# rafaelsoStanford/State_Policy_DiffusionModel

Hardware: AMD Instinct MI355X
Metric: denoise-steps/sec (B=4096, horizon=32) (higher is better)
Workload: dtype f32 (split-fp16 MFMA operands, fp32 accumulate)

## Files before the change

include/spdm.h:

```cpp
#ifndef SPDM_H
#define SPDM_H

#include <stddef.h>
#include <stdint.h>

#ifdef __cplusplus
extern "C" {
#endif

#define SPDM_NAME_MAX 64
#define SPDM_ABI_VERSION 2

typedef enum {
    SPDM_OK = 0,
    SPDM_ERR_INVALID = -1,
    SPDM_ERR_HIP = -2,
    SPDM_ERR_STATE = -3,
    SPDM_ERR_MISSING = -4,
    SPDM_ERR_NOMEM = -5
} spdm_status;

typedef enum { SPDM_DDPM = 0, SPDM_DDIM = 1 } spdm_scheduler_kind;

typedef struct spdm_handle spdm_handle;
// ... 89 lines not shown

typedef struct spdm_encoder spdm_encoder;
int  spdm_encoder_create(int32_t device, const float* h_blob, size_t n_floats, const spdm_tensor_index* h_index,
                         int32_t n_index, spdm_encoder** out);
int  spdm_encoder_forward(spdm_encoder* e, int32_t n_images, const float* d_images, float* d_latent, void* stream);
void spdm_encoder_destroy(spdm_encoder* e);

int  spdm_debug_geometry(int32_t M, int32_t N, int32_t K, int32_t HW, int32_t W, int32_t taps, uint32_t switches,
                         int32_t out[10]);

int  spdm_op_gelu(const float* d_x, float* d_y, size_t n, void* stream);

typedef struct {
    int32_t B, H, W, K, N, taps;
    int32_t split;
    int32_t pro;
    int32_t epi;
    const float* d_src;  int32_t src_ld;
    const float* d_skip; int32_t skip_ld;  int32_t up_C;
    const float* h_weight;
    const double* d_src_stats; int32_t src_slots, src_m_tile, src_n_tiles, src_cnorm;
    const float* d_gamma; const float* d_beta;
    const double* d_skip_stats; int32_t skip_slots, skip_m_tile, skip_n_tiles, skip_cnorm;
    const float* d_skip_gamma; const float* d_skip_beta;
    const float* d_bias; const float* d_resid; int32_t resid_ld;
    float* d_dst; int32_t dst_ld;
    double* d_stats; size_t stats_cap;
    double* d_row_stats; size_t row_stats_cap;
    int32_t out[10];
} spdm_op_gemm_args;

int  spdm_op_gemm(spdm_op_gemm_args* args);

#ifdef __cplusplus
}
#endif
#endif
```

state_policy_diffusionmodel_amd/_lib.py:

```python
from __future__ import annotations

import ctypes
import os
from ctypes import POINTER, c_char_p, c_double, c_float, c_int32, c_int64, c_size_t, c_uint64, c_void_p

from .weights import TensorIndex

HERE = os.path.dirname(os.path.abspath(__file__))
LIB_PATH = os.environ.get("SPDM_LIB") or os.path.join(HERE, "libspdm_hip.so")

SPDM_DDPM, SPDM_DDIM = 0, 1
SPDM_FLAG_DEBUG_KEEP = 1
SPDM_FLAG_EXACT_FP32 = 2
SPDM_FLAG_SIMPLE_UNET = 4
SPDM_FLAG_TRAIN = 8
SPDM_FLAG_TRAIN_ATTENTION = 16
ABI_VERSION = 2


class SpdmOpGemmArgs(ctypes.Structure):
    _fields_ = ([(n, c_int32) for n in ("B", "H", "W", "K", "N", "taps", "split", "pro", "epi")] +
                [("d_src", c_void_p), ("src_ld", c_int32), ("d_skip", c_void_p), ("skip_ld", c_int32), ("up_C", c_int32),
                 ("h_weight", c_void_p),
                 ("d_src_stats", c_void_p)] + [(n, c_int32) for n in ("src_slots", "src_m_tile", "src_n_tiles", "src_cnorm")] +
                [("d_gamma", c_void_p), ("d_beta", c_void_p),
                 ("d_skip_stats", c_void_p)] + [(n, c_int32) for n in ("skip_slots", "skip_m_tile", "skip_n_tiles", "skip_cnorm")] +
                [("d_skip_gamma", c_void_p), ("d_skip_beta", c_void_p),
                 ("d_bias", c_void_p), ("d_resid", c_void_p), ("resid_ld", c_int32),
                 ("d_dst", c_void_p), ("dst_ld", c_int32),
                 ("d_stats", c_void_p), ("stats_cap", c_size_t), ("d_row_stats", c_void_p), ("row_stats_cap", c_size_t),
                 ("out", c_int32 * 10)])


class SpdmConfig(ctypes.Structure):
    _fields_ = [(n, c_int32) for n in ("horizon", "state_dim", "cond_dim", "time_dim", "attention", "max_batch",
                                        "device", "num_train_timesteps", "flags")]


SYMBOLS = {
    "spdm_abi_version": (c_int32, []),
    "spdm_last_error": (c_char_p, []),
    "spdm_create": (c_int32, [POINTER(SpdmConfig), POINTER(c_void_p)]),
    "spdm_destroy": (None, [c_void_p]),
    "spdm_load_weights": (c_int32, [c_void_p, c_void_p, c_size_t, POINTER(TensorIndex), c_int32]),
    "spdm_set_time_table": (c_int32, [c_void_p, c_void_p, c_int32]),
    "spdm_set_schedule": (c_int32, [c_void_p, c_int32, c_int32, c_int32, c_float, c_float]),
    "spdm_set_schedule_tables": (c_int32, [c_void_p, c_int32, c_int32, c_void_p, c_void_p]),
    "spdm_schedule_tables": (c_int32, [c_int32, c_int32, c_int32, c_float, c_float, c_void_p, c_void_p]),
    "spdm_unet_forward": (c_int32, [c_void_p, c_int32, c_void_p, c_void_p, c_int32, c_void_p, c_void_p, c_void_p]),
    "spdm_sample": (c_int32, [c_void_p, c_int32, c_void_p, c_void_p, c_int32, c_int32, c_void_p, c_void_p, c_uint64,
                              c_uint64, c_void_p, c_void_p, c_void_p]),
    "spdm_train_loss_grad": (c_int32, [c_void_p, c_int32, c_void_p, c_void_p, c_int32, c_void_p, c_void_p, c_void_p, c_void_p,
                                       c_void_p, c_void_p, c_void_p]),
    "spdm_sample_begin": (c_int32, [c_void_p, c_int32, c_void_p, c_void_p, c_int32, c_int32, c_void_p, c_void_p,
                                    c_uint64, c_uint64, c_void_p, c_void_p]),
    "spdm_sample_run": (c_int32, [c_void_p, c_int32, c_int32, c_void_p]),
    "spdm_sample_result": (c_int32, [c_void_p, c_void_p, c_void_p]),
    "spdm_graph_captures": (c_int64, [c_void_p]),
    "spdm_debug_tensor": (c_int32, [c_void_p, c_char_p, c_void_p, c_size_t, POINTER(c_int32 * 4)]),
    "spdm_uses_split_precision": (c_int32, [c_void_p]),
    "spdm_demoted_tensors": (c_int32, [c_void_p]),
    "spdm_nonfinite": (c_int32, [c_void_p, POINTER(c_int32), c_void_p]),
    "spdm_set_switch": (c_int32, [c_void_p, c_char_p, c_int32]),
    "spdm_device_bytes": (c_size_t, [c_void_p]),
    "spdm_profile_enable": (c_int32, [c_void_p, c_int32]),
    "spdm_profile_read": (c_int32, [c_void_p, POINTER(c_int64), POINTER(c_double), POINTER(c_double)]),
    "spdm_encoder_create": (c_int32, [c_int32, c_void_p, c_size_t, POINTER(TensorIndex), c_int32, POINTER(c_void_p)]),
    "spdm_encoder_forward": (c_int32, [c_void_p, c_int32, c_void_p, c_void_p, c_void_p]),
    "spdm_encoder_destroy": (None, [c_void_p]),
    "spdm_op_gelu": (c_int32, [c_void_p, c_void_p, c_size_t, c_void_p]),
    "spdm_op_gemm": (c_int32, [POINTER(SpdmOpGemmArgs)]),
    "spdm_debug_geometry": (c_int32, [c_int32] * 6 + [ctypes.c_uint32, POINTER(c_int32 * 10)]),
    "spdm_bench_gemm": (c_int32, [c_int32] * 12 + [POINTER(c_double)]),
}

_lib = None


def load() -> ctypes.CDLL:
    global _lib
    if _lib is not None:
        return _lib
    if not os.path.exists(LIB_PATH):
        raise RuntimeError(
            f"{LIB_PATH} not found: the HIP extension has not been built "
            "(run `python -m state_policy_diffusionmodel_amd.build`); there is no CPU fallback")
    import torch
    lib = ctypes.CDLL(LIB_PATH)
    for name, (res, args) in SYMBOLS.items():
        try:
            fn = getattr(lib, name)
        except AttributeError as e:
            raise RuntimeError(f"{LIB_PATH} does not export {name}") from e
        fn.restype = res
        fn.argtypes = args
    if lib.spdm_abi_version() != ABI_VERSION:
        raise RuntimeError(f"ABI version mismatch: library {lib.spdm_abi_version()}, binding {ABI_VERSION}")
    _lib = lib
    return lib


def check(rc: int, what: str) -> None:
    if rc != 0:
        msg = load().spdm_last_error()
# ... 2 lines not shown
```

state_policy_diffusionmodel_amd/build.py:

```python
from __future__ import annotations

import hashlib
import os
import shutil
import subprocess
import sys
from concurrent.futures import ThreadPoolExecutor

HERE = os.path.dirname(os.path.abspath(__file__))
CSRC = os.path.join(HERE, "csrc")
LIB = os.environ.get("SPDM_BUILD_OUT") or os.path.join(HERE, "libspdm_hip.so")
OBJ = os.path.join(HERE, "csrc", "_obj" + ("_" + os.path.basename(LIB).replace(".", "_") if os.environ.get("SPDM_BUILD_OUT") else ""))
SOURCES = ["conv_gemm.hip", "conv_wide.hip", "conv_skinny.hip", "conv_reg.hip", "elementwise.hip", "attention.hip", "sa_fused.hip", "sa_tail.hip", "encoder.hip", "train.hip", "train_attn.hip", "spdm_api.hip"]
HEADERS = ["kernels.h", "device_utils.h", os.path.join("..", "..", "include", "spdm.h")]
FLAGS = ["--offload-arch=gfx950", "-O3", "-std=c++17", "-fPIC", "-Wall", "-Wno-unused-function"]
if os.environ.get("SPDM_DIAG") == "1":
    FLAGS.append("-DSPDM_DIAG")
FLAGS += os.environ.get("SPDM_EXTRA_FLAGS", "").split()


def _hipcc() -> str:
    for cand in (shutil.which("hipcc"), "/opt/rocm/bin/hipcc"):
        if cand and os.path.exists(cand):
            return cand
    raise RuntimeError("hipcc not found: the MI355X build needs ROCm's hipcc")


def _digest() -> str:
    h = hashlib.sha256()
    h.update(" ".join(FLAGS).encode())
    for f in SOURCES + HEADERS:
        with open(os.path.join(CSRC, f), "rb") as fh:
            h.update(fh.read())
    return h.hexdigest()


def build(force: bool = False, verbose: bool = False) -> str:
    stamp = LIB + ".stamp"
    dig = _digest()
    if not force and os.path.exists(LIB) and os.path.exists(stamp) and open(stamp).read().strip() == dig:
        return LIB
    hipcc = _hipcc()
    os.makedirs(OBJ, exist_ok=True)

    def compile_one(src: str) -> str:
        obj = os.path.join(OBJ, src.replace(".hip", ".o"))
# ... 28 lines not shown
```

state_policy_diffusionmodel_amd/csrc/kernels.h:

```cpp
#pragma once
#include <hip/hip_runtime.h>
#include <stdint.h>
#include <mutex>
#include <set>
#include <utility>
#include <vector>

namespace spdm {

inline hipError_t allow_full_lds(const void* kern) {
    static std::mutex mu;
    static std::set<std::pair<int, const void*>> done;
    int dev = 0;
    hipError_t e = hipGetDevice(&dev);
    if (e != hipSuccess) return e;
    std::lock_guard<std::mutex> lk(mu);
    if (done.count({dev, kern})) return hipSuccess;
    e = hipFuncSetAttribute(kern, hipFuncAttributeMaxDynamicSharedMemorySize, (int)(160 * 1024));
    if (e == hipSuccess) done.insert({dev, kern});
    return e;
}

struct StatsRef {
    const double* p;
    int slots;
    int m_tile;
    int n_tiles;
    int HW;
    double inv_count;
};

__host__ __device__ inline int stats_slots(int HW, int m_tile, int n_tiles) {
    return ((HW + m_tile - 2) / m_tile + 1) * n_tiles;
}

enum : unsigned {
    SW_NO_WIDE = 1u << 0, SW_NO_WIDE128 = 1u << 1, SW_NO_W2 = 1u << 2, SW_NO_T512 = 1u << 3, SW_T512 = 1u << 4,
    SW_T3_BIG = 1u << 5, SW_NO_SMALL_TPI3 = 1u << 6, SW_WIDE_N64_2X2 = 1u << 7, SW_NO_SA_FUSED = 1u << 8,
    SW_NO_SA_TAIL = 1u << 9, SW_ATTN_VALU = 1u << 10, SW_SA_NO_WLDS = 1u << 11, SW_NO_FILM_FOLD = 1u << 12,
    SW_NO_GRAPH = 1u << 13, SW_NO_SPLITK = 1u << 14, SW_ARENA_TRACE = 1u << 15, SW_NO_WIDE_PIPE = 1u << 16, SW_NO_SKINNY = 1u << 17, SW_DEEP = 1u << 18,
    SW_NO_FILM_LOCAL = 1u << 19, SW_NO_FUSED_SRC = 1u << 20, SW_FILM_LOCAL = 1u << 21, SW_PIN_GEOMETRY = 1u << 22, SW_NO_WP4 = 1u << 23, SW_G2 = 1u << 24, SW_NO_WP8 = 1u << 25, SW_NO_SA_HEAD = 1u << 26, SW_SA_HEAD = 1u << 27, SW_NO_REG64 = 1u << 28,
    SW_NO_SA_CROP = 1u << 29, SW_NO_SA_OUTC = 1u << 30,
};
struct SwitchName { const char* env; unsigned bit; };
inline const SwitchName* switch_table(int* n) {
    static const SwitchName t[] = {
        {"SPDM_NO_WIDE", SW_NO_WIDE}, {"SPDM_NO_WIDE128", SW_NO_WIDE128}, {"SPDM_NO_W2", SW_NO_W2}, {"SPDM_NO_T512", SW_NO_T512},
        {"SPDM_T512", SW_T512}, {"SPDM_T3_BIG", SW_T3_BIG}, {"SPDM_NO_SMALL_TPI3", SW_NO_SMALL_TPI3},
        {"SPDM_WIDE_N64_2X2", SW_WIDE_N64_2X2}, {"SPDM_NO_SA_FUSED", SW_NO_SA_FUSED}, {"SPDM_NO_SA_TAIL", SW_NO_SA_TAIL},
        {"SPDM_ATTN_VALU", SW_ATTN_VALU}, {"SPDM_SA_NO_WLDS", SW_SA_NO_WLDS}, {"SPDM_NO_FILM_FOLD", SW_NO_FILM_FOLD},
        {"SPDM_NO_GRAPH", SW_NO_GRAPH}, {"SPDM_NO_SPLITK", SW_NO_SPLITK}, {"SPDM_ARENA_TRACE", SW_ARENA_TRACE}, {"SPDM_NO_WIDE_PIPE", SW_NO_WIDE_PIPE}, {"SPDM_NO_SKINNY", SW_NO_SKINNY}, {"SPDM_DEEP", SW_DEEP},
        {"SPDM_NO_FILM_LOCAL", SW_NO_FILM_LOCAL}, {"SPDM_NO_FUSED_SRC", SW_NO_FUSED_SRC},
        {"SPDM_FILM_LOCAL", SW_FILM_LOCAL}, {"SPDM_PIN_GEOMETRY", SW_PIN_GEOMETRY},
        {"SPDM_NO_WP4", SW_NO_WP4}, {"SPDM_G2", SW_G2}, {"SPDM_NO_WP8", SW_NO_WP8},
        {"SPDM_NO_SA_HEAD", SW_NO_SA_HEAD}, {"SPDM_SA_HEAD", SW_SA_HEAD}, {"SPDM_NO_REG64", SW_NO_REG64},
        {"SPDM_NO_SA_CROP", SW_NO_SA_CROP}, {"SPDM_NO_SA_OUTC", SW_NO_SA_OUTC}};
    *n = (int)(sizeof(t) / sizeof(t[0]));
    return t;
}
unsigned switches_from_env();
int spdm_tune(int idx, int dflt);

enum { PRO_NONE = 0, PRO_GN = 1, PRO_GN_GELU = 2, PRO_POOL = 3, PRO_UPCAT = 4 };
enum { EPI_STATS = 0, EPI_BIAS = 1, EPI_BIAS_GELU = 2, EPI_BIAS_RESID = 3, EPI_PLAIN = 4 };

enum { ROUTE_GEMM = 0, ROUTE_SKINNY = 1, ROUTE_REG = 2, ROUTE_WIDE = 3 };
enum { VAR_PLAIN = 0, VAR_W2 = 1, VAR_WP4 = 2, VAR_WP8 = 3, VAR_PIPE = 4, VAR_G2 = 5 };
struct GemmRoute { int kernel, variant, m_tile, n_tile; };

struct GemmArgs {
    const float* src;  int src_ld;
    const float* wgt;
    int split;
    const float* wgt_frag;
    float* dst;        int dst_ld;
    int M, K, N;
    int geom_M;
    int taps;
    int H, W, HW;
    int pro;  StatsRef pro_stats;  const float* pro_gamma;  const float* pro_beta;
    int up_C;  const float* skip;  int skip_ld;  StatsRef skip_stats;  const float* skip_gamma;  const float* skip_beta;
    int epi;  double* epi_stats;   const float* bias;  const float* resid;  int resid_ld;
    double* row_stats;
    int ksplit;  float* partial;
    unsigned sw;
    int debug;
    unsigned long long* stamps;
    GemmRoute* route;
};
enum { DBG_NO_MFMA = 1, DBG_NO_WLOAD = 2, DBG_NO_GELU = 4, DBG_NO_STORE = 8, DBG_NO_ALOAD = 16, DBG_PP = 64, DBG_STAMP = 128 };

struct GemmGeom {
    int m_tile, n_tile, n_tiles;
    int slots;
    int ksplit;
    int skinny;
    int reg;
    int st_m_tile, st_n_tiles;
};
GemmGeom gemm_geometry(int M, int N, int K, int HW, int W, int taps, int split, unsigned sw, bool stats_epi = false);
GemmGeom gemm_geometry(const GemmArgs& a);
constexpr size_t SPLITK_WORKSPACE_BYTES = (size_t)48 << 20;
__host__ __device__ inline int combine_rows(int HW, int N) {
    int r = HW;
    while ((r & 1) == 0 && (long long)r * N > 2048) r >>= 1;
    return r;
}
bool conv_skinny_geometry(int M, int N, int K, int HW, int W, int taps, int split, unsigned sw, int* m_tile, int* n_tile);
hipError_t launch_conv_skinny(const GemmArgs& a, const GemmGeom& g, hipStream_t s);
bool conv_reg_geometry(int M, int N, int K, int HW, int W, int taps, int split, unsigned sw);
hipError_t launch_conv_reg64(const GemmArgs& a, const GemmGeom& g, hipStream_t s);
hipError_t launch_splitk_combine(const float* partial, int ksplit, float* dst, int M, int N, int HW, double* stats,
                                 hipStream_t s);
hipError_t launch_gemm(const GemmArgs& a, hipStream_t s);
bool gemm_takes_fused_source(const GemmArgs& a);
bool gemm_takes_two_sources(const GemmArgs& a);
double gemm_flops(const GemmArgs& a);
bool conv_wide_supported(const GemmArgs& a, const GemmGeom& g);
hipError_t launch_conv_wide(const GemmArgs& a, const GemmGeom& g, hipStream_t s);

inline std::vector<float> frag_order_weights(const std::vector<float>& split, int taps, int N, int K) {
    std::vector<float> out(split.size());
    const int nch = K / 32, nbn = N / 16;
    for (int t = 0; t < taps; ++t)
        for (int c = 0; c < nch; ++c)
            for (int nb = 0; nb < nbn; ++nb)
                for (int part = 0; part < 2; ++part)
                    for (int kg = 0; kg < 4; ++kg)
                        for (int l16 = 0; l16 < 16; ++l16) {
                            const size_t dst = ((((size_t)(t * nch + c) * nbn + nb) * 2 + part) * 64 + kg * 16 + l16) * 4;
                            const size_t src = ((size_t)t * N + nb * 16 + l16) * K + c * 32 + part * 16 + kg * 4;
                            for (int j = 0; j < 4; ++j) out[dst + j] = split[src + j];
                        }
    return out;
}

int conv_in_parts(int Hp, int Wp, int B);
hipError_t launch_conv_in(const float* x, const float* w , float* dst, double* stats,
                          int B, int H0, int D, int Hp, int Wp, int lh, int lw, int* step_dev, int* t_dev,
                          const int* timesteps_dev, int n_steps, int adv, hipStream_t s, int B_geom = 0);

struct AffineSrc {
    const float* x; int C;
    StatsRef st; const float* gamma; const float* beta;
};
hipError_t launch_pool(const AffineSrc& src, float* dst, int B, int H, int W, hipStream_t s);
hipError_t launch_upcat(const AffineSrc& up, const AffineSrc& skip, float* dst, int B, int Hin, int Win,
                        hipStream_t s);
hipError_t launch_film_apply(const AffineSrc& src, const float* temb_table , const int* t_dev,
                             int t_count, const float* film , float* dst, double* row_stats,
                             int B, int HW, hipStream_t s);
struct FilmSpec {
// ... 105 lines not shown
```

state_policy_diffusionmodel_amd/csrc/spdm_api.hip:

```cpp
#include <hip/hip_runtime.h>

#include <algorithm>
#include <cmath>
#include <cstdarg>
#include <cstdio>
#include <cstdlib>
#include <cstring>
#include <map>
#include <set>
#include <string>
#include <vector>

#include "../../include/spdm.h"
#include "kernels.h"

using namespace spdm;

static thread_local char g_err[512] = "";
static int fail(int code, const char* fmt, ...) {
    va_list ap;
    va_start(ap, fmt);
    vsnprintf(g_err, sizeof(g_err), fmt, ap);
    va_end(ap);
    return code;
// ... 1071 lines not shown
        free(mid);
        return out;
    }
    bool conv_fused(int mode, const Value& src0, const Value* skip, const ConvW& w, int level, const float* gamma,
                    const float* beta, Value* out_v) {
        if (err || !h->split || (h->sw & SW_NO_FUSED_SRC) || h->arena.keep || h->d_partial == nullptr) return false;
        if (dry) {
            if (!((h->dry_fuse_mask >> fuse_slot) & 1)) return false;
            *out_v = conv_out(w, level, dry_geometry(w, level), gamma, beta);
            return true;
        }
        if (!h->weights_loaded || !w.ws || !w.wf) return false;
        const bool upcat = mode == PRO_UPCAT;
        if (upcat ? (!skip || src0.t.C + skip->t.C != w.cin) : src0.t.C != w.cin) return false;
        auto args = [&](const Value* out) {
            return conv_args(w, level, 1, mode, asrc(src0), upcat ? src0.t.C : 0, upcat ? asrc(*skip) : AffineSrc{}, out);
        };
        if (!gemm_takes_fused_source(args(nullptr))) return false;
        *out_v = conv_out(w, level, gemm_geometry(args(nullptr)), gamma, beta);
        if (!err) gemm(args(out_v), "conv3x3 implicit GEMM (fused source)");
        return true;
    }
    bool conv_two(const Tensor& up2x, const Value& skip, const ConvW& w, int level, const float* gamma, const float* beta, Value* out_v) {
        if (!conv_two_ok(up2x.C, skip, w, level)) return false;
        *out_v = conv_out(w, level, dry ? dry_geometry(w, level) : gemm_geometry(two_args(up2x.p, skip, w, level, nullptr)), gamma, beta);
        if (!err && !dry) gemm(two_args(up2x.p, skip, w, level, out_v), "conv3x3 implicit GEMM (two-source input)");
        return true;
    }
    bool conv_two_ok(int C_up, const Value& skip, const ConvW& w, int level) const {
        if (err || !h->split || (h->sw & SW_NO_FUSED_SRC) || h->arena.keep || C_up + skip.t.C != w.cin) return false;
        if (dry) return (h->dry_fuse_mask >> (3 + fuse_slot)) & 1;
        return h->weights_loaded && w.ws && w.wf && gemm_takes_two_sources(two_args(skip.t.p, skip, w, level, nullptr));
    }
    GemmArgs two_args(const float* up, const Value& skip, const ConvW& w, int level, const Value* out) const {
        const int C_up = w.cin - skip.t.C;
        return conv_args(w, level, 1, skip.pending_gn() ? PRO_GN : PRO_NONE, AffineSrc{up, C_up}, C_up, asrc(skip), out);
    }
    StatsBuf row_stats_alloc(int rows, int C, int n_tiles) {
        StatsBuf sb;
        size_t off = 0;
        if (!h->arena.alloc(sizeof(double) * 2 * (size_t)rows * std::max(n_tiles, C / 64), &off)) {
            if (!err) err = fail(SPDM_ERR_NOMEM, "workspace exhausted (batch %d)", B);
            return sb;
        }
        sb.off = off; sb.p = (double*)(h->arena.base + off); sb.valid = true;
        sb.ref.p = sb.p; sb.ref.slots = n_tiles; sb.ref.m_tile = 1 << 30; sb.ref.n_tiles = n_tiles; sb.ref.HW = 1;
        sb.ref.inv_count = 1.0 / (double)C;
        return sb;
    }
    void linear(const float* x, int ld, int rows, const LinW& w, float* y, int epi, const float* resid,
                const StatsBuf* ln = nullptr, const float* ln_g = nullptr, const float* ln_b = nullptr,
                double* row_stats_out = nullptr) {
        if (err || dry) return;
        const AffineSrc src = ln ? AffineSrc{x, ld, ln->ref, ln_g, ln_b} : AffineSrc{x, ld};
        gemm(linear_args(src, rows, (rows / B) * Bg(), w, h->split, h->sw, epi, y, resid, row_stats_out), "linear GEMM");
    }
    bool sa_fused(const AttnW& w, int level) const {
        return h->split && sa_fused_supported(HWl(level), w.C) && !(h->sw & SW_NO_SA_FUSED) && (!h->weights_loaded || w.fw[0]);
    }
    bool sa_crop(const AttnW& w, int level) const {
        return sa_fused(w, level) && !h->arena.keep && !(h->sw & SW_NO_SA_CROP) &&
               sa_crop_supported(HWl(level), w.C, h->cfg.horizon, h->cfg.state_dim);
    }
    bool eps_ready = false;
    Tensor attention(Tensor& x, StatsBuf& xs, const AttnW& w, int level, Tensor* ab = nullptr, const FilmSpec* fs = nullptr,
                     bool final_outc = false) {
// ... 171 lines not shown
        const Tensor y = c.film_attention(b2, h->down[i], i, lout, use_cond, dn[i]);
        c.tap(xn[i], y);
        Value nv;
        nv.t = y;
        cur = nv;
        if (i < 2) skips[i + 1] = nv;
    }
    c.prof_begin();
    Value b1 = c.double_conv(cur, h->bot[0], 3);
    Value b2 = c.double_conv(b1, h->bot[1], 3);
    Value x5 = c.double_conv(b2, h->bot[2], 3);
    c.prof_end();
    c.tap_gn("x5", x5, 3);
    static const char* un[3] = {"u1", "u2", "u3"};
    static const char* an[3] = {"a4", "a5", "a6"};
    cur = x5;
    for (int i = 0; i < 3; ++i) {
        const int lin = 3 - i, lout = 2 - i;
        Value& skip = skips[2 - i];
        Value a, mid;
        c.fuse_slot = 3 + i;
        if (c.conv_fused(PRO_UPCAT, cur, &skip, h->up[i].dc1.first, lout, h->up[i].dc1.gamma, h->up[i].dc1.beta, &mid)) {
            c.free(cur);
            c.free(skip);
            c.prof_begin();
            a = c.conv(mid, h->up[i].dc1.second, lout, true, h->up[i].dc1.gamma, h->up[i].dc1.beta);
            c.free(mid);
        } else if (c.conv_two_ok(cur.t.C, skip, h->up[i].dc1.first, lout)) {
            Tensor u2 = c.talloc(cur.t.C, lout);
            AffineSrc none{};
            if (!c.err && !c.dry) c.check(launch_upcat(c.asrc(cur), none, u2.p, B, c.Hl(lin), c.Wl(lin), c.s), "upsample");
            c.free(cur);
            c.prof_begin();
            if (!c.conv_two(u2, skip, h->up[i].dc1.first, lout, h->up[i].dc1.gamma, h->up[i].dc1.beta, &mid) && !c.err)
                c.err = fail(SPDM_ERR_STATE, "plan: two-source convolution refused after it was offered");
            c.free(u2);
            c.free(skip);
            a = c.conv(mid, h->up[i].dc1.second, lout, true, h->up[i].dc1.gamma, h->up[i].dc1.beta);
            c.free(mid);
        } else {
            Value cat;
            cat.t = c.talloc(cur.t.C + skip.t.C, lout);
            if (!c.err && !c.dry)
                c.check(launch_upcat(c.asrc(cur), c.asrc(skip), cat.t.p, B, c.Hl(lin), c.Wl(lin), c.s), "upsample+concat");
            c.free(cur);
            c.free(skip);
            c.prof_begin();
            a = c.double_conv(cat, h->up[i].dc1, lout);
        }
        Value b3 = c.double_conv(a, h->up[i].dc2, lout);
        c.prof_end();
        const Tensor y = c.film_attention(b3, h->up[i], 3 + i, lout, use_cond, un[i], i == 2);
        c.tap(an[i], y);
        Value nv;
        nv.t = y;
        cur = nv;
    }
    *feat_out = cur.t;
    return c.err;
}

static int plan_simple(Ctx& c, const float* x, Tensor* feat_out) {
    spdm_handle* h = c.h;
    const int B = c.B;
    auto dconv = [&](Tensor& in, const DoubleConvW& w, int level, bool residual) {
        Value vin;
        vin.t = in;
        Value raw = c.double_conv(vin, w, level, true);
        Tensor y = c.talloc(raw.t.C, level);
        if (!c.err && !c.dry) c.check(launch_dc_finish(c.asrc(raw), residual ? in.p : nullptr, y.p, B, c.HWl(level), c.s), "dc_finish");
        c.free(raw);
        c.free(in);
// ... 1041 lines not shown
    if (q.d_skip_stats)
        skip = AffineSrc{q.d_skip, q.skip_ld, ref(q.d_skip_stats, q.skip_slots, q.skip_m_tile, q.skip_n_tiles, HW,
                                                  q.skip_cnorm > 0 ? q.skip_cnorm : q.K - q.up_C), q.d_skip_gamma, q.d_skip_beta};
    const int pro = (two && q.d_skip_stats) ? PRO_GN : q.pro;
    GemmArgs a = gemm_args(M, M, q.H, q.W, q.K, q.N, q.taps, split, sw, (float*)dp, pro, src, q.up_C, skip, (const float*)dw,
                           (const float*)dwf, q.d_dst, q.dst_ld, q.epi, q.epi == EPI_STATS ? q.d_stats : nullptr, q.d_bias,
                           q.d_resid, q.resid_ld, q.d_row_stats);
    if (fused && !gemm_takes_fused_source(a)) {
        release();
        return fail(SPDM_ERR_INVALID, "op_gemm: this launch does not take a fused source (the plan materialises it)");
    }
    if (two && !gemm_takes_two_sources(a)) {
        release();
        return fail(SPDM_ERR_INVALID, "op_gemm: this launch does not take a two-source input (the plan concatenates)");
    }
    GemmRoute r{-1, -1, -1, -1};
    a.route = &r;
    if (q.epi == EPI_STATS) e = hipMemset(q.d_stats, 0xff, (size_t)q.B * g.slots * 2 * sizeof(double));
    if (e == hipSuccess && q.d_row_stats) e = hipMemset(q.d_row_stats, 0xff, (size_t)M * g.n_tiles * 2 * sizeof(double));
    if (e != hipSuccess) { release(); return fail(SPDM_ERR_HIP, "op_gemm: %s", hipGetErrorString(e)); }
    const hipError_t el = launch_gemm(a, nullptr);
    const hipError_t es = hipDeviceSynchronize();
    release();
    if (el != hipSuccess)
        return fail(el == hipErrorInvalidValue && r.kernel < 0 ? SPDM_ERR_INVALID : SPDM_ERR_HIP,
                    "op_gemm: launch_gemm failed (%s) %s; device: %s", hipGetErrorString(el),
                    r.kernel < 0 ? "before any kernel was dispatched (a host-side shape contract)" : "after a kernel was dispatched",
                    hipGetErrorString(es));
    if (es != hipSuccess) return fail(SPDM_ERR_HIP, "op_gemm: %s", hipGetErrorString(es));
    q.out[0] = r.kernel; q.out[1] = r.variant; q.out[2] = r.m_tile; q.out[3] = r.n_tile; q.out[4] = g.ksplit;
    q.out[5] = two ? 1 : 0; q.out[6] = fused ? 1 : 0; q.out[7] = g.slots; q.out[8] = g.st_m_tile; q.out[9] = g.st_n_tiles;
    return SPDM_OK;
}
```

Measured before the change: 519,400.

## Fuse level-0 up-path DoubleConv into one kernel keeping intermediate in LDS

Adds a conv_pair kernel that runs both 3x3 convolutions of the level-0 up-block DoubleConv in a single launch, one block per image. The intermediate activation is GroupNorm-normalized, GELU-applied, split to fp16 hi/lo and kept in LDS, so it never makes a round trip through global memory and needs no separate statistics pass or second launch. It is enabled by default for batches of at least 1024 on the split-precision path, with a switch to disable it. It costs one block per sample at occupancy 1 with large LDS use and a hand-scheduled MFMA pipeline, which may lower latency hiding compared with the tuned generic GEMM kernels.

Result: no change. 524,600, median of 6 (+1.0%).

```diff
diff --git a/include/spdm.h b/include/spdm.h
--- a/include/spdm.h
+++ b/include/spdm.h
@@ -145,6 +145,19 @@
 
 int  spdm_op_gemm(spdm_op_gemm_args* args);
 
+typedef struct {
+    int32_t B, H, W, K, up_C, C_mid, C_out;
+    const float* d_src;  int32_t src_ld;
+    const float* d_skip; int32_t skip_ld;
+    const double* d_st; int32_t st_slots, st_m_tile, st_n_tiles, st_cnorm;
+    const float* d_st_gamma; const float* d_st_beta;
+    const float* h_weight_a; const float* h_weight_b;
+    const float* d_gamma; const float* d_beta;
+    float* d_dst; double* d_stats; size_t stats_cap;
+} spdm_op_dconv_args;
+
+int  spdm_op_dconv(spdm_op_dconv_args* args);
+
 #ifdef __cplusplus
 }
 #endif
diff --git a/state_policy_diffusionmodel_amd/_lib.py b/state_policy_diffusionmodel_amd/_lib.py
--- a/state_policy_diffusionmodel_amd/_lib.py
+++ b/state_policy_diffusionmodel_amd/_lib.py
@@ -30,6 +30,14 @@
                  ("d_dst", c_void_p), ("dst_ld", c_int32),
                  ("d_stats", c_void_p), ("stats_cap", c_size_t), ("d_row_stats", c_void_p), ("row_stats_cap", c_size_t),
                  ("out", c_int32 * 10)])
+
+
+class SpdmOpDconvArgs(ctypes.Structure):
+    _fields_ = ([(n, c_int32) for n in ("B", "H", "W", "K", "up_C", "C_mid", "C_out")] +
+                [("d_src", c_void_p), ("src_ld", c_int32), ("d_skip", c_void_p), ("skip_ld", c_int32),
+                 ("d_st", c_void_p)] + [(n, c_int32) for n in ("st_slots", "st_m_tile", "st_n_tiles", "st_cnorm")] +
+                [("d_st_gamma", c_void_p), ("d_st_beta", c_void_p), ("h_weight_a", c_void_p), ("h_weight_b", c_void_p),
+                 ("d_gamma", c_void_p), ("d_beta", c_void_p), ("d_dst", c_void_p), ("d_stats", c_void_p), ("stats_cap", c_size_t)])
 
 
 class SpdmConfig(ctypes.Structure):
@@ -70,6 +78,7 @@
     "spdm_encoder_destroy": (None, [c_void_p]),
     "spdm_op_gelu": (c_int32, [c_void_p, c_void_p, c_size_t, c_void_p]),
     "spdm_op_gemm": (c_int32, [POINTER(SpdmOpGemmArgs)]),
+    "spdm_op_dconv": (c_int32, [POINTER(SpdmOpDconvArgs)]),
     "spdm_debug_geometry": (c_int32, [c_int32] * 6 + [ctypes.c_uint32, POINTER(c_int32 * 10)]),
     "spdm_bench_gemm": (c_int32, [c_int32] * 12 + [POINTER(c_double)]),
 }
diff --git a/state_policy_diffusionmodel_amd/build.py b/state_policy_diffusionmodel_amd/build.py
--- a/state_policy_diffusionmodel_amd/build.py
+++ b/state_policy_diffusionmodel_amd/build.py
@@ -11,7 +11,7 @@
 CSRC = os.path.join(HERE, "csrc")
 LIB = os.environ.get("SPDM_BUILD_OUT") or os.path.join(HERE, "libspdm_hip.so")
 OBJ = os.path.join(HERE, "csrc", "_obj" + ("_" + os.path.basename(LIB).replace(".", "_") if os.environ.get("SPDM_BUILD_OUT") else ""))
-SOURCES = ["conv_gemm.hip", "conv_wide.hip", "conv_skinny.hip", "conv_reg.hip", "elementwise.hip", "attention.hip", "sa_fused.hip", "sa_tail.hip", "encoder.hip", "train.hip", "train_attn.hip", "spdm_api.hip"]
+SOURCES = ["conv_gemm.hip", "conv_wide.hip", "conv_skinny.hip", "conv_reg.hip", "conv_pair.hip", "elementwise.hip", "attention.hip", "sa_fused.hip", "sa_tail.hip", "encoder.hip", "train.hip", "train_attn.hip", "spdm_api.hip"]
 HEADERS = ["kernels.h", "device_utils.h", os.path.join("..", "..", "include", "spdm.h")]
 FLAGS = ["--offload-arch=gfx950", "-O3", "-std=c++17", "-fPIC", "-Wall", "-Wno-unused-function"]
 if os.environ.get("SPDM_DIAG") == "1":
diff --git a/state_policy_diffusionmodel_amd/csrc/conv_pair.hip b/state_policy_diffusionmodel_amd/csrc/conv_pair.hip
--- /dev/null
+++ b/state_policy_diffusionmodel_amd/csrc/conv_pair.hip
@@ -0,0 +1,310 @@
+#include "device_utils.h"
+
+namespace spdm {
+
+typedef float f32x4 __attribute__((ext_vector_type(4)));
+typedef float f32x2 __attribute__((ext_vector_type(2)));
+typedef _Float16 f16x8 __attribute__((ext_vector_type(8)));
+
+namespace {
+
+constexpr float ACT_SCALE = 16.0f;
+constexpr float DESCALE = 1.0f / 2048.0f;
+constexpr int CK = 32;
+constexpr int NCLS = 8, CROWS = 34;
+constexpr int LDK = 36;
+constexpr int CHUNK_F = NCLS * CROWS * LDK;
+constexpr int CMID = 128, COUT = 128, HWS = 256, NTHR = 512;
+constexpr int OPITCH = 128;
+constexpr size_t LDS_BYTES = (size_t)(CMID / CK) * CHUNK_F * sizeof(float) + 16 * sizeof(double);
+static_assert(HWS * OPITCH <= (CMID / CK) * CHUNK_F, "the output tile re-uses the intermediate's LDS");
+
+__device__ __forceinline__ void split2(float a, float b, float& hi, float& lo) {
+    unsigned h, l;
+    split_pair_f16(a * ACT_SCALE, b * ACT_SCALE, h, l);
+    hi = __builtin_bit_cast(float, h);
+    lo = __builtin_bit_cast(float, l);
+}
+
+template <int PRO, bool TWO>
+__global__ __launch_bounds__(NTHR, 1) void dconv0_kernel(const DconvArgs a) {
+    static_assert(PRO == PRO_NONE || PRO == PRO_GN, "prologue: the source's pending GroupNorm, or none");
+    extern __shared__ __attribute__((aligned(16))) float smem[];
+    double* sred = reinterpret_cast<double*>(smem + (CMID / CK) * CHUNK_F);
+
+    const int tid = threadIdx.x, lane = tid & 63;
+    const int wave = __builtin_amdgcn_readfirstlane(tid >> 6);
+    const int wm = wave >> 1, wn = wave & 1, l16 = lane & 15, kg = lane >> 4;
+    const int b = blockIdx.x;
+    const int K = a.K, nch_a = K / CK;
+
+    for (int i = tid; i < (CMID / CK) * NCLS * 2 * LDK; i += NTHR) {
+        const int img = i / (NCLS * 2 * LDK), r = (i / LDK) % (NCLS * 2), f = i % LDK;
+        smem[img * CHUNK_F + ((r >> 1) * CROWS + (r & 1) * (CROWS - 1)) * LDK + f] = 0.f;
+    }
+
+    const bool left = wm < 2;
+    const int hf = wm & 1;
+    const int sd = left ? -1 : 1;
+    const int cls0 = left ? 0 : NCLS - 1;
+    const int aoff0 = ((cls0 * CROWS + 1 + 16 * hf + l16) * LDK) + kg * 4;
+    const int sstride = (left ? 2 : -2) * CROWS * LDK;
+#define DC_DW(j_) ((j_) == 0 ? 0 : (j_) == 1 ? -sd : sd)
+#define DC_SHIFT(kr_, j_) ((DC_DW(j_) * CROWS + ((kr_) - 1)) * LDK)
+#define DC_WTAP(kr_, j_) (3 * (kr_) + DC_DW(j_) + 1)
+
+    const int srow = tid >> 3, c4 = tid & 7;
+    const int nc0 = TWO ? a.up_C / CK : 0;
+    float mean = 0.f, rstd = 1.f;
+    if (PRO == PRO_GN) sample_mean_rstd(a.pro_stats, b, mean, rstd);
+    f32x4 areg[4];
+    f32x4 g4 = {1.f, 1.f, 1.f, 1.f}, b4 = {0.f, 0.f, 0.f, 0.f};
+    bool ident = true;
+#define DC_LOAD_A(chunk_)                                                                                     \
+    {                                                                                                         \
+        const bool first_ = !TWO || (chunk_) < nc0;                                                           \
+        const int cc_ = first_ ? (chunk_) : (chunk_) - nc0;                                                   \
+        const float* p_ = (first_ ? a.src : a.skip) + cc_ * CK + c4 * 4;                                      \
+        const int ld_ = first_ ? a.src_ld : a.skip_ld;                                                        \
+        _Pragma("unroll") for (int p = 0; p < 4; ++p)                                                         \
+            areg[p] = *reinterpret_cast<const f32x4*>(p_ + (size_t)(b * HWS + p * 64 + srow) * ld_);         \
+        ident = PRO == PRO_NONE || (TWO && first_);                                                           \
+        if (!ident) {                                                                                         \
+            g4 = *reinterpret_cast<const f32x4*>(a.pro_gamma + cc_ * CK + c4 * 4);                            \
+            b4 = *reinterpret_cast<const f32x4*>(a.pro_beta + cc_ * CK + c4 * 4);                             \
+        }                                                                                                     \
+    }
+#define DC_STAGE_A(dst_)                                                                                      \
+    {                                                                                                         \
+        _Pragma("unroll") for (int p = 0; p < 4; ++p) {                                                       \
+            f32x4 v_ = areg[p];                                                                               \
+            if (!ident) {                                                                                     \
+                v_.x = (v_.x - mean) * (rstd * g4.x) + b4.x;                                                  \
+                v_.y = (v_.y - mean) * (rstd * g4.y) + b4.y;                                                  \
+                v_.z = (v_.z - mean) * (rstd * g4.z) + b4.z;                                                  \
+                v_.w = (v_.w - mean) * (rstd * g4.w) + b4.w;                                                  \
+            }                                                                                                 \
+            float h0_, l0_, h1_, l1_;                                                                         \
+            split2(v_.x, v_.y, h0_, l0_);                                                                     \
+            split2(v_.z, v_.w, h1_, l1_);                                                                     \
+            const int r_ = p * 64 + srow;                                              \
+            float* row_ = (dst_) + ((r_ & 7) * CROWS + (r_ >> 3) + 1) * LDK;                                  \
+            *reinterpret_cast<f32x2*>(row_ + c4 * 2) = f32x2{h0_, h1_};                                      \
+            *reinterpret_cast<f32x2*>(row_ + 16 + c4 * 2) = f32x2{l0_, l1_};                                 \
+        }                                                                                                     \
+    }
+
+    f32x4 acc[4][4];
+    f16x8 fbt[2][4][2], fat[2][2];
+#define DC_LOAD_B(slot_, wf_, nch_, chunk_, tap_)                                                             \
+    {                                                                                                         \
+        const float* p_ = (wf_) + (size_t)((tap_) * (nch_) + (chunk_)) * (COUT / 16) * 512;                 \
+        _Pragma("unroll") for (int c_ = 0; c_ < 4; ++c_) {                                                    \
+            fbt[slot_][c_][0] = *reinterpret_cast<const f16x8*>(p_ + c_ * 512);                              \
+            fbt[slot_][c_][1] = *reinterpret_cast<const f16x8*>(p_ + c_ * 512 + 256);                        \
+        }                                                                                                     \
+    }
+#define DC_LOAD_FA(slot_, abuf_, s_, shift_)                                                                  \
+    {                                                                                                         \
+        const float* q_ = (abuf_) + aoff0 + (s_) * sstride + (shift_);                                        \
+        fat[slot_][0] = *reinterpret_cast<const f16x8*>(q_);                                                  \
+        fat[slot_][1] = *reinterpret_cast<const f16x8*>(q_ + 16);                                             \
+    }
+#define DC_CHUNK(abuf_, wf_, nch_, chunk_, nchunk_)                                                           \
+    {                                                                                                         \
+        int g_ = 0;                                                                                           \
+        _Pragma("unroll") for (int T = 0; T < 9; ++T) {                                                       \
+            const int kr = T / 3, j = T % 3;                                                                  \
+            if (T < 8) { DC_LOAD_B((T + 1) & 1, wf_, nch_, chunk_, DC_WTAP((T + 1) / 3, (T + 1) % 3)) }       \
+            else { DC_LOAD_B(1, wf_, nch_, nchunk_, DC_WTAP(0, 0)) }                                          \
+            _Pragma("unroll") for (int s = (j == 2 ? 1 : 0); s < 4; ++s) {                                    \
+                if (s < 3) { DC_LOAD_FA((g_ + 1) & 1, abuf_, s + 1, DC_SHIFT(kr, j)) }                        \
+                else if (T < 8) { DC_LOAD_FA((g_ + 1) & 1, abuf_, ((T + 1) % 3 == 2) ? 1 : 0, DC_SHIFT((T + 1) / 3, (T + 1) % 3)) } \
+                __builtin_amdgcn_sched_barrier(0);                                                            \
+                _Pragma("unroll") for (int c = 0; c < 4; ++c)                                                 \
+                    acc[s][c] = __builtin_amdgcn_mfma_f32_16x16x32_f16(fat[g_ & 1][0], fbt[T & 1][c][0], acc[s][c], 0, 0, 0); \
+                _Pragma("unroll") for (int c = 0; c < 4; ++c)                                                 \
+                    acc[s][c] = __builtin_amdgcn_mfma_f32_16x16x32_f16(fat[g_ & 1][0], fbt[T & 1][c][1], acc[s][c], 0, 0, 0); \
+                _Pragma("unroll") for (int c = 0; c < 4; ++c)                                                 \
+                    acc[s][c] = __builtin_amdgcn_mfma_f32_16x16x32_f16(fat[g_ & 1][1], fbt[T & 1][c][0], acc[s][c], 0, 0, 0); \
+                __builtin_amdgcn_sched_barrier(0);                                                            \
+                ++g_;                                                                                         \
+            }                                                                                                 \
+        }                                                                                                     \
+        _Pragma("unroll") for (int c = 0; c < 4; ++c) { fbt[0][c][0] = fbt[1][c][0]; fbt[0][c][1] = fbt[1][c][1]; } \
+    }
+
+    const float* wfa = a.wf_a + (size_t)(wn * 4 * 2) * 256 + lane * 4;
+    const float* wfb = a.wf_b + (size_t)(wn * 4 * 2) * 256 + lane * 4;
+#pragma unroll
+    for (int s = 0; s < 4; ++s)
+#pragma unroll
+        for (int c = 0; c < 4; ++c) acc[s][c] = f32x4{0.f, 0.f, 0.f, 0.f};
+
+    DC_LOAD_B(0, wfa, nch_a, 0, DC_WTAP(0, 0))
+    DC_LOAD_A(0)
+    DC_STAGE_A(smem)
+    __syncthreads();
+    DC_LOAD_FA(0, smem, 0, DC_SHIFT(0, 0))
+    for (int chunk = 0; chunk < nch_a; ++chunk) {
+        const bool more = chunk + 1 < nch_a;
+        const float* abuf = smem + (chunk & 1) * CHUNK_F;
+        if (more) { DC_LOAD_A(chunk + 1) }
+        DC_CHUNK(abuf, wfa, nch_a, chunk, (more ? chunk + 1 : chunk))
+        if (more) {
+            DC_STAGE_A(smem + ((chunk + 1) & 1) * CHUNK_F)
+            __syncthreads();
+            DC_LOAD_FA(0, smem + ((chunk + 1) & 1) * CHUNK_F, 0, DC_SHIFT(0, 0))
+        }
+    }
+    DC_LOAD_B(0, wfb, CMID / CK, 0, DC_WTAP(0, 0))
+
+    {
+        float s1 = 0.f, s2 = 0.f;
+#pragma unroll
+        for (int s = 0; s < 4; ++s)
+#pragma unroll
+            for (int c = 0; c < 4; ++c) {
+                acc[s][c] *= DESCALE;
+#pragma unroll
+                for (int r = 0; r < 4; ++r) { s1 += acc[s][c][r]; s2 += acc[s][c][r] * acc[s][c][r]; }
+            }
+        const double d1 = wave_sum_f64((double)s1), d2 = wave_sum_f64((double)s2);
+        if (lane == 0) { sred[wave * 2] = d1; sred[wave * 2 + 1] = d2; }
+    }
+    __syncthreads();
+    {
+        double t1 = 0.0, t2 = 0.0;
+        for (int w8 = 0; w8 < 8; ++w8) { t1 += sred[w8 * 2]; t2 += sred[w8 * 2 + 1]; }
+        const double inv = 1.0 / ((double)CMID * HWS);
+        const double m = t1 * inv;
+        double var = t2 * inv - m * m;
+        if (var < 0.0) var = 0.0;
+        const float mu = (float)m, rs = (float)(1.0 / sqrt(var + 1e-5));
+        const bool odd = (l16 & 1) != 0;
+#pragma unroll
+        for (int c = 0; c < 4; ++c) {
+            const int n = wn * 64 + c * 16 + l16;
+            const float gs = rs * a.gamma[n], bt = a.beta[n];
+            float* img = smem + (size_t)(n >> 5) * CHUNK_F + ((n & 31) >> 1);
+#pragma unroll
+            for (int s = 0; s < 4; ++s) {
+                float v[4];
+#pragma unroll
+                for (int r = 0; r < 4; ++r) v[r] = gelu_erf((acc[s][c][r] - mu) * gs + bt);
+                const int cls = cls0 + (left ? 2 * s : -2 * s);
+                float* rowb = img + (cls * CROWS + 1 + 16 * hf + 4 * kg) * LDK;
+#pragma unroll
+                for (int rp = 0; rp < 4; rp += 2) {
+                    const float send = odd ? v[rp] : v[rp + 1];
+                    const float recv = __builtin_bit_cast(float, __builtin_amdgcn_update_dpp(0, __builtin_bit_cast(int, send), 0xB1, 0xf, 0xf, false));
+                    float hi, lo;
+                    if (odd) split2(recv, v[rp + 1], hi, lo);
+                    else split2(v[rp], recv, hi, lo);
+                    float* row = rowb + (rp + (odd ? 1 : 0)) * LDK;
+                    row[0] = hi;
+                    row[16] = lo;
+                }
+            }
+        }
+#pragma unroll
+        for (int s = 0; s < 4; ++s)
+#pragma unroll
+            for (int c = 0; c < 4; ++c) acc[s][c] = f32x4{0.f, 0.f, 0.f, 0.f};
+    }
+    __syncthreads();
+
+    DC_LOAD_FA(0, smem, 0, DC_SHIFT(0, 0))
+    for (int chunk = 0; chunk < CMID / CK; ++chunk) {
+        const float* abuf = smem + chunk * CHUNK_F;
+        const int nxt = min(chunk + 1, CMID / CK - 1);
+        DC_CHUNK(abuf, wfb, CMID / CK, chunk, nxt)
+        if (chunk + 1 < CMID / CK) { DC_LOAD_FA(0, smem + (chunk + 1) * CHUNK_F, 0, DC_SHIFT(0, 0)) }
+    }
+#undef DC_LOAD_A
+#undef DC_STAGE_A
+#undef DC_LOAD_B
+#undef DC_LOAD_FA
+#undef DC_CHUNK
+#undef DC_DW
+#undef DC_SHIFT
+#undef DC_WTAP
+
+    {
+        float s1 = 0.f, s2 = 0.f;
+#pragma unroll
+        for (int s = 0; s < 4; ++s)
+#pragma unroll
+            for (int c = 0; c < 4; ++c) {
+                acc[s][c] *= DESCALE;
+#pragma unroll
+                for (int r = 0; r < 4; ++r) { s1 += acc[s][c][r]; s2 += acc[s][c][r] * acc[s][c][r]; }
+            }
+        const double d1 = wave_sum_f64((double)s1), d2 = wave_sum_f64((double)s2);
+        if (lane == 0) { sred[wave * 2] = d1; sred[wave * 2 + 1] = d2; }
+    }
+    __syncthreads();
+    float* otile = smem;
+#pragma unroll
+    for (int s = 0; s < 4; ++s) {
+        const int cls = cls0 + (left ? 2 * s : -2 * s);
+#pragma unroll
+        for (int c = 0; c < 4; ++c) {
+            const int n = wn * 64 + c * 16 + l16;
+#pragma unroll
+            for (int r = 0; r < 4; ++r) {
+                const int p = (16 * hf + 4 * kg + r) * 8 + cls;
+                otile[p * OPITCH + (n ^ (((p >> 5) & 3) << 4))] = acc[s][c][r];
+            }
+        }
+    }
+    if (tid == 0) {
+        double t1 = 0.0, t2 = 0.0;
+        for (int w8 = 0; w8 < 8; ++w8) { t1 += sred[w8 * 2]; t2 += sred[w8 * 2 + 1]; }
+        double* o = a.stats + (size_t)b * a.stats_slots * 2;
+        o[0] = t1;
+        o[1] = t2;
+    }
+    __syncthreads();
+    {
+        const int c4o = tid & 31, r0 = tid >> 5;
+#pragma unroll 4
+        for (int p = 0; p < HWS / 16; ++p) {
+            const int row = p * 16 + r0;
+            const f32x4 v = *reinterpret_cast<const f32x4*>(otile + row * OPITCH + ((c4o * 4) ^ (((row >> 5) & 3) << 4)));
+            *reinterpret_cast<f32x4*>(a.dst + (size_t)(b * HWS + row) * COUT + c4o * 4) = v;
+        }
+    }
+}
+
+template <int PRO, bool TWO>
+hipError_t launch_cfg(const DconvArgs& a, hipStream_t s) {
+    auto kern = dconv0_kernel<PRO, TWO>;
+    if (hipError_t e = allow_full_lds(reinterpret_cast<const void*>(kern)); e != hipSuccess) return e;
+    hipLaunchKernelGGL(kern, dim3(a.B), dim3(NTHR), LDS_BYTES, s, a);
+    return hipGetLastError();
+}
+
+}
+
+bool dconv0_supported(int H, int W, int K, int C_mid, int C_out, int up_C) {
+    return H * W == HWS && W == 8 && C_mid == CMID && C_out == COUT && K % CK == 0 && K >= CK && up_C % CK == 0 && up_C >= 0 &&
+           up_C < K;
+}
+
+hipError_t launch_dconv0(const DconvArgs& a, hipStream_t s) {
+    if (!dconv0_supported(a.H, a.W, a.K, a.C_mid, a.C_out, a.skip ? a.up_C : 0) || a.B <= 0 || a.stats_slots < 1) return hipErrorInvalidValue;
+    if (!a.src || !a.wf_a || !a.wf_b || !a.gamma || !a.beta || !a.dst || !a.stats) return hipErrorInvalidValue;
+    const bool two = a.skip != nullptr;
+    if (a.src_ld % 4 || a.src_ld < (two ? a.up_C : a.K) || (two && (a.skip_ld % 4 || a.skip_ld < a.K - a.up_C || a.up_C <= 0)))
+        return hipErrorInvalidValue;
+    if (a.pro != PRO_NONE && (a.pro != PRO_GN || !a.pro_stats.p || !a.pro_gamma || !a.pro_beta)) return hipErrorInvalidValue;
+    if (two) return a.pro == PRO_GN ? launch_cfg<PRO_GN, true>(a, s) : launch_cfg<PRO_NONE, true>(a, s);
+    return a.pro == PRO_GN ? launch_cfg<PRO_GN, false>(a, s) : launch_cfg<PRO_NONE, false>(a, s);
+}
+
+double dconv0_flops(const DconvArgs& a) {
+    return 2.0 * a.B * HWS * 9.0 * ((double)a.K * a.C_mid + (double)a.C_mid * a.C_out);
+}
+
+}
diff --git a/state_policy_diffusionmodel_amd/csrc/kernels.h b/state_policy_diffusionmodel_amd/csrc/kernels.h
--- a/state_policy_diffusionmodel_amd/csrc/kernels.h
+++ b/state_policy_diffusionmodel_amd/csrc/kernels.h
@@ -40,7 +40,7 @@
     SW_NO_SA_TAIL = 1u << 9, SW_ATTN_VALU = 1u << 10, SW_SA_NO_WLDS = 1u << 11, SW_NO_FILM_FOLD = 1u << 12,
     SW_NO_GRAPH = 1u << 13, SW_NO_SPLITK = 1u << 14, SW_ARENA_TRACE = 1u << 15, SW_NO_WIDE_PIPE = 1u << 16, SW_NO_SKINNY = 1u << 17, SW_DEEP = 1u << 18,
     SW_NO_FILM_LOCAL = 1u << 19, SW_NO_FUSED_SRC = 1u << 20, SW_FILM_LOCAL = 1u << 21, SW_PIN_GEOMETRY = 1u << 22, SW_NO_WP4 = 1u << 23, SW_G2 = 1u << 24, SW_NO_WP8 = 1u << 25, SW_NO_SA_HEAD = 1u << 26, SW_SA_HEAD = 1u << 27, SW_NO_REG64 = 1u << 28,
-    SW_NO_SA_CROP = 1u << 29, SW_NO_SA_OUTC = 1u << 30,
+    SW_NO_SA_CROP = 1u << 29, SW_NO_SA_OUTC = 1u << 30, SW_NO_DC0 = 1u << 31,
 };
 struct SwitchName { const char* env; unsigned bit; };
 inline const SwitchName* switch_table(int* n) {
@@ -54,7 +54,7 @@
         {"SPDM_FILM_LOCAL", SW_FILM_LOCAL}, {"SPDM_PIN_GEOMETRY", SW_PIN_GEOMETRY},
         {"SPDM_NO_WP4", SW_NO_WP4}, {"SPDM_G2", SW_G2}, {"SPDM_NO_WP8", SW_NO_WP8},
         {"SPDM_NO_SA_HEAD", SW_NO_SA_HEAD}, {"SPDM_SA_HEAD", SW_SA_HEAD}, {"SPDM_NO_REG64", SW_NO_REG64},
-        {"SPDM_NO_SA_CROP", SW_NO_SA_CROP}, {"SPDM_NO_SA_OUTC", SW_NO_SA_OUTC}};
+        {"SPDM_NO_SA_CROP", SW_NO_SA_CROP}, {"SPDM_NO_SA_OUTC", SW_NO_SA_OUTC}, {"SPDM_NO_DC0", SW_NO_DC0}};
     *n = (int)(sizeof(t) / sizeof(t[0]));
     return t;
 }
@@ -118,6 +118,19 @@
 double gemm_flops(const GemmArgs& a);
 bool conv_wide_supported(const GemmArgs& a, const GemmGeom& g);
 hipError_t launch_conv_wide(const GemmArgs& a, const GemmGeom& g, hipStream_t s);
+
+struct DconvArgs {
+    const float* src;  int src_ld;
+    const float* skip; int skip_ld; int up_C;
+    int pro;  StatsRef pro_stats;  const float* pro_gamma;  const float* pro_beta;
+    const float* wf_a; const float* wf_b;
+    const float* gamma; const float* beta;
+    float* dst; double* stats; int stats_slots;
+    int B, H, W, K, C_mid, C_out;
+};
+bool dconv0_supported(int H, int W, int K, int C_mid, int C_out, int up_C);
+hipError_t launch_dconv0(const DconvArgs& a, hipStream_t s);
+double dconv0_flops(const DconvArgs& a);
 
 inline std::vector<float> frag_order_weights(const std::vector<float>& split, int taps, int N, int K) {
     std::vector<float> out(split.size());
diff --git a/state_policy_diffusionmodel_amd/csrc/spdm_api.hip b/state_policy_diffusionmodel_amd/csrc/spdm_api.hip
--- a/state_policy_diffusionmodel_amd/csrc/spdm_api.hip
+++ b/state_policy_diffusionmodel_amd/csrc/spdm_api.hip
@@ -1127,6 +1127,34 @@
         if (dry) return (h->dry_fuse_mask >> (3 + fuse_slot)) & 1;
         return h->weights_loaded && w.ws && w.wf && gemm_takes_two_sources(two_args(skip.t.p, skip, w, level, nullptr));
     }
+    static constexpr int DC0_MIN_BATCH = 1024;
+    bool dc0_ok(int C_up, const Value& skip, const DoubleConvW& w, int level) const {
+        if (err || dry || !h->split || (h->sw & SW_NO_DC0) || h->arena.keep || Bg() < DC0_MIN_BATCH || !h->weights_loaded) return false;
+        if (!w.first.ws || !w.first.wf || !w.second.ws || !w.second.wf) return false;
+        if (w.first.taps != 9 || w.second.taps != 9 || w.second.cin != w.first.cout || C_up + skip.t.C != w.first.cin) return false;
+        return dconv0_supported(Hl(level), Wl(level), w.first.cin, w.first.cout, w.second.cout, C_up);
+    }
+    Value dc0_two(const Tensor& up2x, const Value& skip, const DoubleConvW& w, int level) {
+        Value out;
+        out.t = talloc(w.second.cout, level);
+        out.st = salloc(HWl(level), w.second.cout, HWl(level), 1);
+        out.gamma = w.gamma; out.beta = w.beta;
+        if (err) return out;
+        DconvArgs a{};
+        a.src = up2x.p; a.src_ld = up2x.C;
+        a.skip = skip.t.p; a.skip_ld = skip.t.C; a.up_C = up2x.C;
+        a.pro = skip.pending_gn() ? PRO_GN : PRO_NONE;
+        if (skip.pending_gn()) { a.pro_stats = skip.st.ref; a.pro_gamma = skip.gamma; a.pro_beta = skip.beta; }
+        a.wf_a = w.first.wf; a.wf_b = w.second.wf; a.gamma = w.gamma; a.beta = w.beta;
+        a.dst = out.t.p; a.stats = out.st.p; a.stats_slots = out.st.ref.slots;
+        a.B = B; a.H = Hl(level); a.W = Wl(level); a.K = w.first.cin; a.C_mid = w.first.cout; a.C_out = w.second.cout;
+        if (h->prof && h->prof_open >= 0) {
+            h->prof_evts[h->prof_open].flops += dconv0_flops(a);
+            h->prof_evts[h->prof_open].launches += 1;
+        }
+        check(launch_dconv0(a, s), "level-0 DoubleConvolution (conv_pair)");
+        return out;
+    }
     GemmArgs two_args(const float* up, const Value& skip, const ConvW& w, int level, const Value* out) const {
         const int C_up = w.cin - skip.t.C;
         return conv_args(w, level, 1, skip.pending_gn() ? PRO_GN : PRO_NONE, AffineSrc{up, C_up}, C_up, asrc(skip), out);
@@ -1364,12 +1392,18 @@
             if (!c.err && !c.dry) c.check(launch_upcat(c.asrc(cur), none, u2.p, B, c.Hl(lin), c.Wl(lin), c.s), "upsample");
             c.free(cur);
             c.prof_begin();
-            if (!c.conv_two(u2, skip, h->up[i].dc1.first, lout, h->up[i].dc1.gamma, h->up[i].dc1.beta, &mid) && !c.err)
-                c.err = fail(SPDM_ERR_STATE, "plan: two-source convolution refused after it was offered");
-            c.free(u2);
-            c.free(skip);
-            a = c.conv(mid, h->up[i].dc1.second, lout, true, h->up[i].dc1.gamma, h->up[i].dc1.beta);
-            c.free(mid);
+            if (c.dc0_ok(u2.C, skip, h->up[i].dc1, lout)) {
+                a = c.dc0_two(u2, skip, h->up[i].dc1, lout);
+                c.free(u2);
+                c.free(skip);
+            } else {
+                if (!c.conv_two(u2, skip, h->up[i].dc1.first, lout, h->up[i].dc1.gamma, h->up[i].dc1.beta, &mid) && !c.err)
+                    c.err = fail(SPDM_ERR_STATE, "plan: two-source convolution refused after it was offered");
+                c.free(u2);
+                c.free(skip);
+                a = c.conv(mid, h->up[i].dc1.second, lout, true, h->up[i].dc1.gamma, h->up[i].dc1.beta);
+                c.free(mid);
+            }
         } else {
             Value cat;
             cat.t = c.talloc(cur.t.C + skip.t.C, lout);
@@ -2477,3 +2511,49 @@
     q.out[5] = two ? 1 : 0; q.out[6] = fused ? 1 : 0; q.out[7] = g.slots; q.out[8] = g.st_m_tile; q.out[9] = g.st_n_tiles;
     return SPDM_OK;
 }
+
+extern "C" int spdm_op_dconv(spdm_op_dconv_args* p) {
+    if (!p) return fail(SPDM_ERR_INVALID, "op_dconv: null argument");
+    const spdm_op_dconv_args& q = *p;
+    const bool two = q.d_skip != nullptr;
+    if (q.B <= 0 || !dconv0_supported(q.H, q.W, q.K, q.C_mid, q.C_out, two ? q.up_C : 0) || (two && q.up_C <= 0))
+        return fail(SPDM_ERR_INVALID, "op_dconv: unsupported shape (32 x 8 maps, C_mid == C_out == 128, K %% 32 == 0)");
+    if (!q.d_src || !q.d_dst || !q.d_stats || !q.h_weight_a || !q.h_weight_b || !q.d_gamma || !q.d_beta)
+        return fail(SPDM_ERR_INVALID, "op_dconv: src, dst, stats, weights, gamma and beta are required");
+    if (q.stats_cap < (size_t)q.B * 2) return fail(SPDM_ERR_INVALID, "op_dconv: statistics buffer needs %d doubles", 2 * q.B);
+    if (q.src_ld % 4 || q.src_ld < (two ? q.up_C : q.K) || (two && (q.skip_ld % 4 || q.skip_ld < q.K - q.up_C)))
+        return fail(SPDM_ERR_INVALID, "op_dconv: bad leading dimension");
+    if (q.d_st && (!q.d_st_gamma || !q.d_st_beta || q.st_slots <= 0 || q.st_m_tile <= 0 || q.st_n_tiles <= 0))
+        return fail(SPDM_ERR_INVALID, "op_dconv: pending GroupNorm needs gamma, beta and the partials' geometry");
+    const std::vector<float> wa = Loader::conv_taps(q.h_weight_a, q.C_mid, q.K, 9), wb = Loader::conv_taps(q.h_weight_b, q.C_out, q.C_mid, 9);
+    if (!Loader::split_range_ok(wa) || !Loader::split_range_ok(wb))
+        return fail(SPDM_ERR_INVALID, "op_dconv: weights outside the split format's range (the loader keeps such a layer on the exact path)");
+    const std::vector<float> fa = frag_order_weights(Loader::split_format(wa), 9, q.C_mid, q.K);
+    const std::vector<float> fb = frag_order_weights(Loader::split_format(wb), 9, q.C_out, q.C_mid);
+    void* dfa = nullptr;
+    void* dfb = nullptr;
+    hipError_t e = hipMalloc(&dfa, fa.size() * 4);
+    if (e == hipSuccess) e = hipMalloc(&dfb, fb.size() * 4);
+    if (e == hipSuccess) e = hipMemcpy(dfa, fa.data(), fa.size() * 4, hipMemcpyHostToDevice);
+    if (e == hipSuccess) e = hipMemcpy(dfb, fb.data(), fb.size() * 4, hipMemcpyHostToDevice);
+    DconvArgs a{};
+    a.src = q.d_src; a.src_ld = q.src_ld;
+    if (two) { a.skip = q.d_skip; a.skip_ld = q.skip_ld; a.up_C = q.up_C; }
+    a.pro = q.d_st ? PRO_GN : PRO_NONE;
+    if (q.d_st) {
+        const int cnorm = q.st_cnorm > 0 ? q.st_cnorm : (two ? q.K - q.up_C : q.K);
+        a.pro_stats = StatsRef{q.d_st, q.st_slots, q.st_m_tile, q.st_n_tiles, q.H * q.W, 1.0 / ((double)cnorm * q.H * q.W)};
+        a.pro_gamma = q.d_st_gamma; a.pro_beta = q.d_st_beta;
+    }
+    a.wf_a = (const float*)dfa; a.wf_b = (const float*)dfb; a.gamma = q.d_gamma; a.beta = q.d_beta;
+    a.dst = q.d_dst; a.stats = q.d_stats; a.stats_slots = 1;
+    a.B = q.B; a.H = q.H; a.W = q.W; a.K = q.K; a.C_mid = q.C_mid; a.C_out = q.C_out;
+    hipError_t el = hipSuccess;
+    if (e == hipSuccess) el = launch_dconv0(a, nullptr);
+    const hipError_t es = hipDeviceSynchronize();
+    (void)hipFree(dfa);
+    (void)hipFree(dfb);
+    if (e != hipSuccess || el != hipSuccess || es != hipSuccess)
+        return fail(SPDM_ERR_HIP, "op_dconv: %s / %s / %s", hipGetErrorString(e), hipGetErrorString(el), hipGetErrorString(es));
+    return SPDM_OK;
+}
```
